# foobaz/pngloss

Measured on AMD Instinct MI355X. Metric: Mpixels/s (filter+quantise path), 4096x4096 RGBA8 s=19; bit-exact vs ref, higher is better.
Workload: dtype u8

## Files before the change

pngloss_amd/csrc/pl_seg_core.h:

```cpp
#ifndef PL_SEG_CORE_H
#define PL_SEG_CORE_H

#include <stdint.h>
#include <stddef.h>
#include <string.h>

#include "pl_result.h"

#if defined(__HIPCC__)
#define PLS_HD __host__ __device__ __forceinline__
#else
#define PLS_HD inline
#endif

#if defined(__HIP_DEVICE_COMPILE__)
#define PLS_THREADS(tid, nt) for (int tid = (int)threadIdx.x, pls_once_ = 1; pls_once_ && tid < (int)(nt); pls_once_ = 0)
#define PLS_SYNC() __syncthreads()
#define PLS_ATOMIC_ADD(p, v) atomicAdd((p), (v))
#define PLS_ATOMIC_MIN(p, v) atomicMin((p), (v))
#define PLS_ATOMIC_OR(p, v) atomicOr((p), (v))
#define PLS_ATOMIC_CAS(p, cmp, v) atomicCAS((p), (cmp), (v))
#define PLS_ATOMIC_ADD_RET(p, v) atomicAdd((p), (v))
#define PLS_ATOMIC_EXCH(p, v) atomicExch((p), (v))
#define PLS_ATOMIC_ADD64(p, v) atomicAdd((unsigned long long *)(p), (unsigned long long)(v))
#define PLS_CLOCK() wall_clock64()
#define PLS_ATOMIC_MAX(p, v) atomicMax((p), (v))
#define PLS_WAVE_LEADER(tid) (((tid) & 63) == 0)
__device__ __forceinline__ uint32_t pls_wave_sum_u32(uint32_t v) { for (int o = 32; o > 0; o >>= 1) v += __shfl_xor(v, o, 64); return v; }
__device__ __forceinline__ uint64_t pls_wave_sum_u64(uint64_t v) { for (int o = 32; o > 0; o >>= 1) v += __shfl_xor(v, o, 64); return v; }
__device__ __forceinline__ int pls_wave_max_i(int v) { for (int o = 32; o > 0; o >>= 1) { const int t = __shfl_xor(v, o, 64); v = t > v ? t : v; } return v; }
__device__ __forceinline__ int pls_wave_min_i(int v) { for (int o = 32; o > 0; o >>= 1) { const int t = __shfl_xor(v, o, 64); v = t < v ? t : v; } return v; }
#define PLS_ATOMIC_MAX_I(p, v) atomicMax((p), (v))
#define PLS_ATOMIC_MAX_U(p, v) atomicMax((p), (v))
#define PLS_ATOMIC_MIN_I(p, v) atomicMin((p), (v))
#define PLS_HOST_VISIBLE_ADD(p, v) __hip_atomic_fetch_add((p), (v), __ATOMIC_RELAXED, __HIP_MEMORY_SCOPE_SYSTEM)
#define PLS_HOST_VISIBLE_STORE(p, v) __hip_atomic_store((p), (v), __ATOMIC_RELAXED, __HIP_MEMORY_SCOPE_SYSTEM)
#else
#define PLS_THREADS(tid, nt) for (int tid = 0; tid < (int)(nt); ++tid)
#define PLS_SYNC() ((void)0)
#define PLS_ATOMIC_ADD(p, v) (*(p) += (v))
#define PLS_ATOMIC_MIN(p, v) (*(p) = *(p) < (v) ? *(p) : (v))
#define PLS_ATOMIC_OR(p, v) (*(p) |= (v))
inline uint32_t pls_host_cas(uint32_t *p, uint32_t cmp, uint32_t v) { const uint32_t old = *p; if (old == cmp) *p = v; return old; }
inline uint32_t pls_host_add_ret(uint32_t *p, uint32_t v) { const uint32_t old = *p; *p += v; return old; }
#define PLS_ATOMIC_CAS(p, cmp, v) pls_host_cas((p), (cmp), (v))
#define PLS_ATOMIC_ADD_RET(p, v) pls_host_add_ret((p), (v))
#define PLS_ATOMIC_EXCH(p, v) (*(p) = (v))
#define PLS_ATOMIC_ADD64(p, v) (*(p) += (v))
#define PLS_CLOCK() 0ull
#define PLS_ATOMIC_MAX(p, v) (*(p) = *(p) > (v) ? *(p) : (v))
#define PLS_WAVE_LEADER(tid) (true)
inline uint32_t pls_wave_sum_u32(uint32_t v) { return v; }
inline uint64_t pls_wave_sum_u64(uint64_t v) { return v; }
inline int pls_wave_max_i(int v) { return v; }
inline int pls_wave_min_i(int v) { return v; }
#define PLS_ATOMIC_MAX_I(p, v) (*(p) = *(p) > (v) ? *(p) : (v))
#define PLS_ATOMIC_MAX_U(p, v) (*(p) = *(p) > (v) ? *(p) : (v))
#define PLS_ATOMIC_MIN_I(p, v) (*(p) = *(p) < (v) ? *(p) : (v))
#define PLS_HOST_VISIBLE_ADD(p, v) (*(p) += (v))
#define PLS_HOST_VISIBLE_STORE(p, v) (*(p) = (v))
#endif

#if defined(__HIP_DEVICE_COMPILE__) && !defined(SEG_PLAIN_POINTERS)
#define SEG_AS_LDS __attribute__((address_space(3)))
#define SEG_AS_GLB __attribute__((address_space(1)))
#else
#define SEG_AS_LDS
#define SEG_AS_GLB
#endif
typedef SEG_AS_LDS uint32_t *seg_lds_u32;
typedef SEG_AS_LDS uint8_t *seg_lds_u8;
typedef SEG_AS_LDS uint16_t *seg_lds_u16;

#if defined(__HIPCC__)
#define PLS_UNROLL _Pragma("unroll")
#else
#define PLS_UNROLL
#endif
#define SEG_NFILT 5
#ifndef SEG_DEBUG_ROW
#define SEG_DEBUG_ROW(kind, failed, winner, start_none)
#endif
#ifndef SEG_DEBUG_REPAIR
#define SEG_DEBUG_REPAIR(f, c, sg, est, sid)
#endif
#ifndef SEG_DEBUG_BREAK
#define SEG_DEBUG_BREAK(f, c, sg, est, y)
#endif
#ifndef SEG_DEBUG_STATE
#define SEG_DEBUG_STATE(f, k, sl, i, ps)
// ... 609 lines not shown
    return true;
}
inline bool seg_build_params(SegParams &P, int strength, int bleed, bool force_seeded = false)
{
    memset(&P, 0, sizeof P);
    if (strength < 0 || strength > 255 || bleed < 1 || bleed > 32767) return false;
    P.strength = strength; P.bleed = bleed; P.unit = 1; P.tparts = SEG_TPARTS;
    for (int d = -256; d <= 255; d++) {
        const SegSplit s = seg_split_slow(d, bleed);
        P.lut_a[d + 256] = ((uint32_t)s.rem & 0xffffu) | ((uint32_t)s.h << 16);
        P.lut_b[d + 256] = ((uint32_t)s.t & 255u) | (((uint32_t)s.f & 255u) << 8) | (((uint32_t)s.v & 255u) << 16) | ((uint32_t)s.h << 24);
    }
    {
        int rm_ = 0, tm_ = 0;
        for (int D = 0; D < 256; D++) {
            const SegSplit a = seg_split_slow(D, bleed), b = seg_split_slow(-D, bleed);
            rm_ = seg_max(rm_, seg_max(seg_abs(a.rem), seg_abs(b.rem))); tm_ = seg_max(tm_, seg_max(seg_abs(a.h), seg_abs(b.h)));
            P.rt_max[D] = (uint8_t)seg_min(255, rm_ + tm_);
        }
    }
    int rmax = 0, tmax = 0;
    for (int d = -strength; d <= strength; d++) { const SegSplit s = seg_split_slow(d, bleed); if (seg_abs(s.rem) > rmax) rmax = seg_abs(s.rem); if (seg_abs(s.h) > tmax) tmax = seg_abs(s.h); }
    P.cmax = rmax + tmax; P.tmax = tmax; P.dmax = strength + P.cmax;
    if (!force_seeded && seg_build_exhaustive(P, strength, bleed)) return true;
    P.seeded = 1; P.kin = P.cmax <= 12 ? (bleed == 1 ? 20 : 16) : (P.cmax <= 24 ? 24 : SEG_KIN);
    P.ns = 0; P.nsp = 64; P.keyn = 0; P.ns_small = 0; P.small_ok = 0; P.idx0_big = P.idx0_small = (uint32_t)SEG_INVALID;
    if (P.cmax > 127 || tmax > 127 || 2 * P.cmax + 1 > SEG_NSP) return false;
    int tstep = 1;
    while ((2 * P.cmax + 1) * (2 * (tmax / tstep) + 1) > SEG_NSP) tstep++;
    int n = 0;
    for (int cn = -P.cmax; cn <= P.cmax; cn++)
        for (int th = -(tmax / tstep) * tstep; th <= tmax; th += tstep) P.seed_small[n++] = (uint32_t)(cn + 128) | ((uint32_t)(th + 128) << 8);
    P.nseed_small = n;
    return true;
}


#define SEG_SM_ENUM (SEG_TBL_WORDS * 4 + 2048 + SEG_SMALL_SEGS * SEG_L * 4 * 8 + 64 + 4 * 512 * 4 + 4 * 512 * 2 + 4 * SEG_NSP * 4 + 4 * SEG_NSP * 2 + SEG_THREADS * 2 + SEG_THREADS * 4 + 64)
#define SEG_SM_ENUM_NT(nt) (SEG_TBL_WORDS * 4 + (SEG_L + 1) * 4 * 8 + 2048 + 32 + 4 * SEG_HT * 4 + 4 * SEG_HT * 2 + 4 * SEG_NSP * 4 + 4 * SEG_NSP * 2 + (nt) * 2 + (nt) * 4 + 128)
#define SEG_SM_REPLAY (4096 + SEG_TBL_WORDS * 4 + SEG_GRP * SEG_L * 4 * 8 + SEG_GRP * 256 + SEG_GRP * SEG_PARTS * 4 * 8 + SEG_GRP * SEG_L * 16 + (SEG_GRP * SEG_L + 3) * 4 + 64)
#ifndef SEG_WATCH_OF
#define SEG_WATCH_OF(V) ((V) > 8 ? 2 : 8)
#endif
#define SEG_SM_POST_V(V) ((768 + ((V) + 1) * 256 + ((V) * SEG_L + 2) * 4 + 64 + 512 + 2 * ((V) * SEG_L + 2) + 2 * (V) * SEG_L + 32 + 64 + (V) * SEG_L + (V) * (SEG_L + 1) + SEG_WATCH_OF(V) * ((V) * (SEG_L + 1) + 8) + 2 * 20 * 4 + 512 + 64) * 4)
#define SEG_SM_POST SEG_SM_POST_V(SEG_VGRP)
#define SEG_SM_CTLVAL_V(V) (SEG_SM_CTL > SEG_SM_POST_V(V) ? SEG_SM_CTL : SEG_SM_POST_V(V))
#define SEG_SM_CTLVAL SEG_SM_CTLVAL_V(SEG_VGRP)
#define SEG_SM_CTL ((8 + 512 + (sizeof(SegCtl) + 7) / 8 * 2 + (sizeof(SegAcc) + 7) / 8 * 2 + 56 + SEG_NFILT * (SEG_COMMIT_W + 4) * 4 + SEG_COMMIT_W * 4 + (SEG_NFILT + 1) * 256 + 16) * 4)
static_assert((1024 + SEG_TBL_WORDS) * 4 <= SEG_SM_CTL, "a candidate workgroup of the control kernel (histograms + table staging) fits the commit workgroups' request");

PLS_HD void seg_cnt_add(uint32_t *cnt, int bin, uint32_t v) { PLS_ATOMIC_ADD(&cnt[bin >> 2], v << (8 * (bin & 3))); }
PLS_HD uint32_t seg_cnt_get(const uint32_t *cnt, int bin) { return (cnt[bin >> 2] >> (8 * (bin & 3))) & 255u; }
static_assert(SEG_L * 4 <= 255, "a segment's bump count of a bin fits a byte");
template <int F, bool TRX, int N = 0>
PLS_HD int seg_steps(const SegPix *px, int pstride, int n, SegState &st, const SegStepMem &M, const SegGeo &g, uint32_t *out, uint32_t *cnt)
{
    const int nn = N > 0 ? N : n;
    int bad = 0;
    if (nn <= 0) return 0;
    SegPix p = px[0];
    for (int k = 0; k < nn; k++) {
        const SegPix pn = px[(size_t)(k + 1 < nn ? k + 1 : k) * pstride];
        const uint32_t w = seg_step_fast<F, TRX>(p, st, bad, M, g);
        if (out) out[(size_t)k * 4] = w;
        if (cnt) seg_cnt_add(cnt, seg_cand_bin(w), 1u);
        p = pn;
    }
    return bad;
}
template <int F, bool TRX, int N = 0>
PLS_HD int seg_run_fast(const SegPix *px, int pstride, int n, SegState &st, seg_lds_cu32 tw, const SegGeo &g, seg_lds_cu32 lut)
{
    return seg_bad(seg_steps<F, TRX, N>(px, pstride, n, st, seg_step_mem(tw, lut), g, nullptr, nullptr)) ? 1 : 0;
}
template <bool TRX, int N = 0>
PLS_HD int seg_run_fast_t(int f, const SegPix *px, int pstride, int n, SegState &st, seg_lds_cu32 tw, const SegGeo &g, seg_lds_cu32 lut)
{
    switch (f) {
    case 1: return seg_run_fast<1, TRX, N>(px, pstride, n, st, tw, g, lut);
    case 2: return seg_run_fast<2, TRX, N>(px, pstride, n, st, tw, g, lut);
    case 3: return seg_run_fast<3, TRX, N>(px, pstride, n, st, tw, g, lut);
    case 4: return seg_run_fast<4, TRX, N>(px, pstride, n, st, tw, g, lut);
    default: return seg_run_fast<0, TRX, N>(px, pstride, n, st, tw, g, lut);
    }
}
PLS_HD int seg_run_fast_f(int f, bool trx, const SegPix *px, int pstride, int n, SegState &st, seg_lds_cu32 tw, const SegGeo &g, seg_lds_cu32 lut)
{
    return trx ? seg_run_fast_t<true>(f, px, pstride, n, st, tw, g, lut) : seg_run_fast_t<false>(f, px, pstride, n, st, tw, g, lut);
}
template <int N>
PLS_HD int seg_run_fast_f(int f, bool trx, const SegPix *px, int pstride, SegState &st, seg_lds_cu32 tw, const SegGeo &g, seg_lds_cu32 lut)
{
    static_assert(N > 0, "a compile-time count of steps");
    return trx ? seg_run_fast_t<true, N>(f, px, pstride, N, st, tw, g, lut) : seg_run_fast_t<false, N>(f, px, pstride, N, st, tw, g, lut);
}

#define SEG_K1 4
#ifndef SEG_K1_ONE_CHUNK
#define SEG_K1_ONE_CHUNK 4
#endif
PLS_HD int seg_k1(int ns) { return ns <= SEG_NSP ? SEG_K1_ONE_CHUNK : SEG_K1; }
#define SEG_HT 512
template <int NT, int K1>
PLS_HD void seg_enum_body_k(const SegJob &j, const SegParams &P, const SegCtlView &cv, int par, int f, int seg, int chalf, unsigned char *smem)
{
    static_assert(K1 > 0 && K1 < SEG_PL, "the dedupe lies inside the first part");
    if (cv.finished || cv.active != 1) return;
    const uint32_t W = j.W, bpp = j.bpp;
    constexpr int NCH = NT / SEG_NSP;
    const int c0 = chalf * NCH;
    if ((uint32_t)c0 >= bpp) return;
    const uint32_t x0 = (uint32_t)seg * SEG_L;
    if (x0 >= W) return;
    if (cv.start_x && x0 <= cv.start_x) return;
    uint32_t *tw = (uint32_t *)smem;
    SegPix *px = (SegPix *)(smem + SEG_TBL_WORDS * 4);
    uint32_t *lut = (uint32_t *)(px + (SEG_L + 1) * 4);
    uint32_t *trflag = lut + 512;
// ... 709 lines not shown
        }
        PLS_SYNC();
        PLS_THREADS(tid, NT) {
            const uint32_t total2 = misc[64 + NC];
            if ((uint32_t)tid < total2) {
                int k = 0;
                PLS_UNROLL
                for (int q = 1; q < NC; q++) k += (uint32_t)tid >= misc[64 + q] ? 1 : 0;
                const uint32_t i = (uint32_t)tid - misc[64 + k], cq = q0 + (uint32_t)k, u = cq / bpp, c = cq % bpp;
                SegState st = seg_state_unpack(pool2[misc[32 + k] + i]);
                const SegPix *pk = px + (size_t)k * NPX;
                const uint32_t sg0 = u * E, nsg = seg_umin(E, nseg - sg0);
                int bad = 0;
                for (uint32_t sl = 1; sl < nsg; sl++) {
                    const size_t slot = (((size_t)f * nseg + sg0 + sl) * 4 + c) * SEG_NSP + i;
                    for (int part = 0; part < SEG_PARTS; part++) {
                        if (part) j.rck[slot * (SEG_PARTS - 1) + (part - 1)] = bad ? 0xFFFFFFFFu : seg_state_pack(st);
                        bad |= seg_run_fast_f(f, trx, pk + 1 + sl * SEG_L + part * SEG_PL, 1, SEG_PL, st, SEG_LDS_CU32(tw), G, SEG_LDS_CU32(lut));
                    }
                    j.rst[slot] = bad ? 0xFFFFFFFFu : seg_state_pack(st);
                    SEG_DEBUG_STATE(f, (long)cv.y * 100000 + (long)cq, sl, i, bad ? 0xFFFFFFFFu : seg_state_pack(st));
                    if (sl + 1 == nsg) j.rout[slot] = (uint16_t)(bad ? (uint32_t)SEG_INVALID : seg_any_encode(P, f, pk[(sl + 1) * SEG_L], st));
                }
            }
        }
    }
    if (prof) {
        PLS_SYNC();
        PLS_THREADS(tid, NT) {
            if (tid == 0) {
                te[4] = PLS_CLOCK();
                for (int q = 0; q < PLR_SEG_ENUM_PHASES; q++) { PLS_ATOMIC_MAX(&j.result[PLR_SEG_ENUM_MAX + q], (int32_t)(te[q + 1] - te[q])); PLS_ATOMIC_ADD((uint32_t *)&j.result[PLR_SEG_ENUM_SUM + q], (uint32_t)(te[q + 1] - te[q])); }
                PLS_ATOMIC_ADD((uint32_t *)&j.result[PLR_SEG_ENUM_RUNS], 1u);
                PLS_ATOMIC_ADD((uint32_t *)&j.result[PLR_SEG_ENUM_STATES], 4u * misc[32 + NC] / (uint32_t)NC);
            }
        }
    }
}

PLS_HD bool seg_unit_from_seeds(const SegJob &j, const SegParams &P, const SegCtlView &cv, int f, int seeds)
{
    return seeds != 0 && P.seed_n > 0 && !seg_is_small(P, f) && cv.start_x == 0u && j.nbreak * 16u <= cv.y + 128u;
}

PLS_HD void seg_load_frozen(const SegJob &j, int par, int f, uint32_t *Hf, uint32_t *rank, int tid, int nt)
{
    for (int b = tid; b < 256; b += nt) {
        Hf[b] = j.H0[par * 256 + b] + j.base[((size_t)par * SEG_NFILT + f) * 256 + b];
        rank[b] = j.orig_rank[f * 256 + b];
    }
}

PLS_HD void seg_walk(int f, const SegPix *px, int pstride, uint32_t xa, uint32_t xe, SegState &st, seg_lds_cu32 tw, seg_lds_cu32 lut, const uint32_t *Hf,
                     const uint32_t *rank, const SegGeo &G, const uint32_t *lut_g, int bleed, uint32_t *out, uint32_t *cnt)
{
    const SegState st0 = st;
    int bad = 0;
    const SegStepMem M = seg_step_mem(tw, lut);
    const int n = xa < xe ? (int)(xe - xa) : 0;
    switch (f) {
    case 1: bad = seg_steps<1, true>(px, pstride, n, st, M, G, out, cnt); break;
    case 2: bad = seg_steps<2, true>(px, pstride, n, st, M, G, out, cnt); break;
    case 3: bad = seg_steps<3, true>(px, pstride, n, st, M, G, out, cnt); break;
    case 4: bad = seg_steps<4, true>(px, pstride, n, st, M, G, out, cnt); break;
    default: bad = seg_steps<0, true>(px, pstride, n, st, M, G, out, cnt); break;
    }
    if (seg_bad(bad)) {
        if (cnt && out) for (uint32_t x = xa; x < xe; x++) seg_cnt_add(cnt, seg_cand_bin(out[(size_t)(x - xa) * 4]), 0u - 1u);
        st = st0;
        for (uint32_t x = xa; x < xe; x++) {
            const uint32_t w = seg_step_scan(f, px[(size_t)(x - xa) * pstride], st, Hf, nullptr, rank, G, lut_g, bleed);
            if (out) out[(size_t)(x - xa) * 4] = w;
            if (cnt) seg_cnt_add(cnt, seg_cand_bin(w), 1u);
        }
    }
}

template <int NT, bool UNITS>
PLS_HD void seg_first_body(const SegJob &j, const SegParams &P, const SegCtlView &cv, int par, int f, unsigned char *smem)
{
    const SegCtl &ctl = j.ctl[par];
    if (cv.finished || cv.active != 1) return;
    const uint32_t W = j.W, bpp = j.bpp, nseg = j.nseg;
    const uint32_t sx = cv.start_x;
    if (sx >= W || sx == 0) return;
    const uint32_t first = sx / SEG_L;
    if (first + 1 >= nseg) return;
    const uint32_t E = UNITS ? seg_unit_of(P, f) : 1u, ulast = seg_umin((first / E) * E + E - 1u, nseg - 1u);
    const uint32_t wend = seg_umin(ulast, nseg - 2u);
    const uint32_t npix = (wend - first + 1u) * SEG_L;
    uint32_t *tw = (uint32_t *)smem;
    uint32_t *lut = tw + SEG_TBL_WORDS;
    uint32_t *Hf = lut + 512, *rank = Hf + 256;
    SegPix *px = (SegPix *)(rank + 256);
    const unsigned long long tf0 = (P.engine_flags & 1) ? PLS_CLOCK() : 0ull;
    const uint32_t y = cv.y;
    const uint32_t *row = seg_row_orig(j, y), *nab = y ? j.img + (size_t)(y - 1u) * W : nullptr, *e0g = seg_e0(j, y);
    const SegGeo G = seg_geo((int)cv.s);
    PLS_THREADS(tid, NT) {
        constexpr int NTW = (SEG_TBL_WORDS + NT - 1) / NT;
        uint32_t vt[NTW], vl = 0, vh = 0, vb = 0, vr = 0;
        SegPixRaw vp = seg_pix_raw_zero();
        PLS_UNROLL
        for (int q = 0; q < NTW; q++) { const int i = tid + q * NT; vt[q] = i < SEG_TBL_WORDS ? j.tables[(size_t)f * SEG_TBL_WORDS + i] : 0u; }
        if (tid < 512) vl = P.lut_a[tid];
        if (tid < 256) { const int b = tid; vh = j.H0[par * 256 + b]; vb = j.base[((size_t)par * SEG_NFILT + f) * 256 + b]; vr = j.orig_rank[f * 256 + b]; }
        static_assert(256 + SEG_UNIT * SEG_L <= NT, "a unit's pixels are staged by the threads behind the first 256");
        if (tid >= 256 && (uint32_t)(tid - 256) < npix) vp = seg_pix_fetch(row, nab, e0g, first * SEG_L + (uint32_t)(tid - 256), W);
        PLS_UNROLL
        for (int q = 0; q < NTW; q++) { const int i = tid + q * NT; if (i < SEG_TBL_WORDS) tw[i] = vt[q]; }
        if (tid < 512) lut[tid] = vl;
        if (tid < 256) { Hf[tid] = vh + vb; rank[tid] = vr; }
        if (tid >= 256 && (uint32_t)(tid - 256) < npix) seg_pix_split4(px + (tid - 256) * 4, vp, bpp, first * SEG_L + (uint32_t)(tid - 256), W);
    }
    PLS_SYNC();
    PLS_THREADS(tid, NT) {
        if (tid < 4 && (uint32_t)tid < bpp) {
            const int c = tid;
            SegState st = seg_state_unpack(ctl.state[f][c]);
            for (uint32_t sg = first; sg <= wend; sg++) {
                const uint32_t xa = sg == first ? sx : sg * SEG_L, xe = (sg + 1u) * SEG_L;
                seg_walk(f, px + (xa - first * SEG_L) * 4 + c, 4, xa, xe, st, SEG_LDS_CU32(tw), SEG_LDS_CU32(lut), Hf, rank, G, lut, P.bleed, nullptr, nullptr);
                if (sg + 1u <= ulast) {
                    j.entry[((size_t)f * nseg + sg + 1u) * 4 + c] = seg_state_pack(st);
                    j.dnout[((size_t)f * nseg + sg + 1u) * 4 + c] = (uint16_t)SEG_INVALID;
                }
// ... 440 lines not shown
PLS_HD int seg_none_reach(const SegJob &j, const SegParams &P, int s, int M, int m);

template <int CT>
PLS_HD void seg_extremes_body(const SegJob &j, const SegParams &P, const SegCtlView &cv, int par, unsigned char *smem)
{
    if (cv.finished || !j.rowmm) return;
    const uint32_t W = j.W, bpp = j.bpp, y = cv.y;
    const uint32_t *row = seg_row_orig(j, y), *e0g = seg_e0(j, y);
    uint32_t *mm = (uint32_t *)smem;
    PLS_THREADS(tid, CT) { if (tid == 0) { mm[0] = 0x80000000u ^ (uint32_t)(-(1 << 30)); mm[1] = 0x80000000u ^ (uint32_t)(1 << 30); } }
    PLS_SYNC();
    PLS_THREADS(tid, CT) {
        int vmax = -(1 << 30), vmin = 1 << 30;
        for (uint32_t x0 = (uint32_t)tid; x0 < W; x0 += 4u * CT) {
            uint32_t o[4], ea[4], eb[4];
            PLS_UNROLL
            for (int q = 0; q < 4; q++) { const uint32_t x = seg_umin(x0 + (uint32_t)q * CT, W - 1u); o[q] = row[x]; ea[q] = e0g[2 * (size_t)x]; eb[q] = e0g[2 * (size_t)x + 1]; }
            PLS_UNROLL
            for (int q = 0; q < 4; q++) {
                const uint32_t e[2] = { ea[q], eb[q] };
                const bool alpha0 = (bpp & 1u) == 0u && ((o[q] >> (8u * (bpp - 1u))) & 255u) == 0u;
                for (uint32_t c = 0; c < bpp; c++) {
                    if (alpha0 && c == bpp - 1u) continue;
                    const int v = (int)((o[q] >> (8 * c)) & 255u) + seg_err_plane(e, seg_plane_of_channel(bpp, (int)c));
                    vmax = seg_max(vmax, v); vmin = seg_min(vmin, v);
                }
            }
        }
        vmax = pls_wave_max_i(vmax); vmin = pls_wave_min_i(vmin);
        if (PLS_WAVE_LEADER(tid)) { PLS_ATOMIC_MAX_U(&mm[0], 0x80000000u ^ (uint32_t)vmax); PLS_ATOMIC_MIN(&mm[1], 0x80000000u ^ (uint32_t)vmin); }
    }
    PLS_SYNC();
    PLS_THREADS(tid, CT) { if (tid == 0) { SEG_AS_GLB int32_t *rmm = seg_rowmm(j, y); rmm[0] = (int)(mm[0] ^ 0x80000000u); rmm[1] = (int)(mm[1] ^ 0x80000000u); } }
}

template <int RNT>
PLS_HD void seg_replay_body(const SegJob &j, const SegParams &P, const SegCtlView &cv, int par, int f, int grp, unsigned char *smem)
{
    const SegCtl &ctl = j.ctl[par];
    if (cv.finished) return;
    const bool lazy = f == 0 && cv.active == 2;
    if (!lazy && cv.active != 1) return;
    const uint32_t W = j.W, bpp = j.bpp, nseg = j.nseg;
    const uint32_t sx = cv.start_x;
    const uint32_t first = sx / SEG_L;
    const uint32_t seg0 = (uint32_t)grp * SEG_GRP, x0g = seg0 * SEG_L;
    const bool walk = !lazy && sx < W && seg0 + SEG_GRP > first;
    uint32_t *Hf = (uint32_t *)smem, *rank = Hf + 256, *lut = Hf + 512, *tw = Hf + 1024;
    SegPix *px = (SegPix *)(tw + SEG_TBL_WORDS);
    uint32_t *cnt = (uint32_t *)(px + SEG_GRP * SEG_L * 4);
    uint32_t *lane = cnt + SEG_GRP * 64;
    uint32_t *cwl = lane + SEG_GRP * SEG_PARTS * 4 * 2;
    uint32_t *oaL = cwl + SEG_REPLAY_THREADS * 4;
    uint32_t *rm = tw;
    uint32_t *red = rm + 768;
    uint32_t *h0s = red + 16;
    const uint32_t y = cv.y;
    const uint32_t *row = seg_row_orig(j, y), *nab = y ? j.img + (size_t)(y - 1u) * W : nullptr, *e0g = seg_e0(j, y);
    const uint32_t *oab = y ? seg_row_orig(j, y - 1u) : nullptr;
    const SegGeo G = seg_geo((int)cv.s);
    const bool adaptive = !j.row_filters || y == 0;
    PLS_THREADS(tid, RNT) {
        const bool walker = walk && tid < SEG_GRP * SEG_PARTS * 4;
        const int sl = tid / (SEG_PARTS * 4), part = (tid >> 2) % SEG_PARTS, c = tid & 3;
        const uint32_t sg = seg0 + (uint32_t)sl;
        const bool live = walker && sg < nseg && sg >= first && (uint32_t)c < bpp;
        const size_t sc = ((size_t)f * nseg + (live ? sg : 0u)) * 4 + c;
        const uint32_t d = live ? (uint32_t)j.dnout[sc] : SEG_INVALID;
        constexpr int NTW = (SEG_TBL_WORDS + RNT - 1) / RNT;
        uint32_t vt[NTW], vl = 0, vh = 0, vb = 0, vr = 0;
        PLS_UNROLL
        for (int q = 0; q < NTW; q++) { const int i = tid + q * RNT; vt[q] = (walk && i < SEG_TBL_WORDS) ? j.tables[(size_t)f * SEG_TBL_WORDS + i] : 0u; }
        if (walk && tid < 512) vl = P.lut_a[tid];
        if (walk && tid < 256) { vh = j.H0[par * 256 + tid]; vb = j.base[((size_t)par * SEG_NFILT + f) * 256 + tid]; vr = j.orig_rank[f * 256 + tid]; }
        const bool pixlane = tid < SEG_REPLAY_THREADS;
        const uint32_t x = pixlane ? x0g + (uint32_t)tid : W;
        const SegPixRaw vp = seg_pix_fetch(row, nab, e0g, x, W);
        const uint32_t voa = (!lazy && oab && x < W) ? oab[x] : 0u;
        uint32_t voa0 = 0, vol0 = 0;
        SegVec16 vw, vw0; vw.a = vw.b = vw.c = vw.d = 0u; vw0 = vw;
        if (!lazy && tid == 0 && x0g) { voa0 = oab ? oab[x0g - 1] : 0u; vol0 = row[x0g - 1]; if (x0g <= sx) vw0 = *(const SEG_AS_GLB SegVec16 *)(j.cand + ((size_t)f * W + x0g - 1) * 4); }
        if (!lazy && x < W && (x < sx || !walk)) vw = *(const SEG_AS_GLB SegVec16 *)(j.cand + ((size_t)f * W + x) * 4);
        uint32_t ck[SEG_PARTS - 1], ent = 0;
        PLS_UNROLL
        for (int q = 0; q < SEG_PARTS - 1; q++) ck[q] = 0xFFFFFFFFu;
        if (live) {
            if (d != SEG_INVALID && d < SEG_NSP) {
                PLS_UNROLL
                for (int q = 0; q < SEG_PARTS - 1; q++) ck[q] = j.rck[(sc * SEG_NSP + d) * (SEG_PARTS - 1) + q];
            }
            if (part == 0) ent = sg == first ? ctl.state[f][c] : j.entry[sc];
        }
        uint32_t st0 = 0, range = 0xFFFFFFFFu;
        if (live) {
            const uint32_t x0 = sg * SEG_L, xend = (uint32_t)seg_min((int)(x0 + SEG_L), (int)W);
            bool mine = part == 0;
            uint32_t xa = sg == first ? sx : x0;
            if (part == 0) st0 = ent;
            else {
                uint32_t ckp = 0xFFFFFFFFu;
                PLS_UNROLL
                for (int q = 0; q < SEG_PARTS - 1; q++) if (q == part - 1) ckp = ck[q];
                if (ckp != 0xFFFFFFFFu && x0 + (uint32_t)part * SEG_PL < xend && x0 + (uint32_t)part * SEG_PL > xa) { mine = true; st0 = ckp; xa = x0 + (uint32_t)part * SEG_PL; }
            }
            if (mine) {
                uint32_t xe = xend;
                PLS_UNROLL
                for (int q = SEG_PARTS - 1; q >= 1; q--)
                    if (q > part && ck[q - 1] != 0xFFFFFFFFu && x0 + (uint32_t)q * SEG_PL < xend && x0 + (uint32_t)q * SEG_PL > xa) xe = x0 + (uint32_t)q * SEG_PL;
                range = (xa - x0g) | ((xe - x0g) << 16);
                SEG_DEBUG_COUNT(part ? 1 : 0, xe - xa);
            }
        }
        if (tid < SEG_GRP * SEG_PARTS * 4) { lane[2 * tid] = st0; lane[2 * tid + 1] = range; }
        if (walk) {
            PLS_UNROLL
            for (int q = 0; q < NTW; q++) { const int i = tid + q * RNT; if (i < SEG_TBL_WORDS) tw[i] = vt[q]; }
            if (tid < 512) lut[tid] = vl;
            if (tid < 256) { Hf[tid] = vh + vb; rank[tid] = vr; }
            for (int i = tid; i < SEG_GRP * 64; i += RNT) cnt[i] = 0u;
        }
        if (pixlane) {
            seg_pix_split4(px + tid * 4, vp, bpp, x, W);
            oaL[tid + 1] = voa;
            cwl[tid * 4 + 0] = vw.a; cwl[tid * 4 + 1] = vw.b; cwl[tid * 4 + 2] = vw.c; cwl[tid * 4 + 3] = vw.d;
        }
        if (tid == 0) {
            oaL[0] = voa0; oaL[SEG_REPLAY_THREADS + 1] = vol0;
            oaL[SEG_REPLAY_THREADS + 2] = (vw0.a & 255u) | ((vw0.b & 255u) << 8) | ((vw0.c & 255u) << 16) | ((vw0.d & 255u) << 24);
        }
    }
    PLS_SYNC();
    if (walk) {
        PLS_THREADS(tid, RNT) {
            if (tid < SEG_GRP * SEG_PARTS * 4 && lane[2 * tid + 1] != 0xFFFFFFFFu) {
                const int sl = tid / (SEG_PARTS * 4), c = tid & 3;
                SegState st = seg_state_unpack(lane[2 * tid]);
                const uint32_t ra = lane[2 * tid + 1] & 0xffffu, re = lane[2 * tid + 1] >> 16;
                seg_walk(f, px + ra * 4 + c, 4, x0g + ra, x0g + re, st, SEG_LDS_CU32(tw), SEG_LDS_CU32(lut), Hf, rank, G, lut, P.bleed, cwl + ra * 4 + c, cnt + sl * 64);
            }
        }
        PLS_SYNC();
    }
    SegAcc &A = j.acc[par];
    PLS_THREADS(tid, RNT) { if (tid < 16) red[tid] = tid == 14 ? (0x80000000u ^ (uint32_t)(-(1 << 30))) : (tid == 15 ? (0x80000000u ^ (uint32_t)(1 << 30)) : 0u); }
    PLS_SYNC();
    {
        PLS_THREADS(tid, RNT) {
            if (walk && tid >= RNT - SEG_REPLAY_THREADS && tid < RNT - SEG_REPLAY_THREADS + 256) {
                const int b = tid - (RNT - SEG_REPLAY_THREADS);
                uint32_t tot = 0, cvs[SEG_GRP];
                PLS_UNROLL
                for (int sl = 0; sl < SEG_GRP; sl++) cvs[sl] = seg_cnt_get(cnt + sl * 64, b);
                PLS_UNROLL
                for (int sl = 0; sl < SEG_GRP; sl++) {
                    const uint32_t sg = seg0 + (uint32_t)sl;
                    if (sg < nseg && sg >= first) { j.segcnt[((size_t)f * nseg + sg) * 256 + b] = (uint16_t)cvs[sl]; tot += cvs[sl]; }
                }
                j.grpcnt[((size_t)f * j.ngrp + grp) * 256 + b] = tot;
            }
            const uint32_t x = (!lazy && tid < SEG_REPLAY_THREADS) ? x0g + (uint32_t)tid : W;
            uint64_t derr = 0; uint32_t hs[SEG_NFILT] = { 0, 0, 0, 0, 0 };
            if (x < W) {
                SegVec16 w; w.a = cwl[tid * 4 + 0]; w.b = cwl[tid * 4 + 1]; w.c = cwl[tid * 4 + 2]; w.d = cwl[tid * 4 + 3];
                if (walk && x >= sx) *(SEG_AS_GLB SegVec16 *)(j.cand + ((size_t)f * W + x) * 4) = w;
                uint32_t lw[4];
                if (tid) { PLS_UNROLL for (int c = 0; c < 4; c++) lw[c] = cwl[(tid - 1) * 4 + c] & 255u; }
                else {
                    uint32_t l0 = 0;
                    if (x0g && x0g <= sx) l0 = oaL[SEG_REPLAY_THREADS + 2];
                    else if (x0g) {
                        for (uint32_t c = 0; c < bpp; c++) l0 |= (walk ? (lane[2 * c] & 255u) : 0u) << (8 * c);
                        j.grpleft[(size_t)f * j.ngrp + grp] = l0;
                    }
                    PLS_UNROLL for (int c = 0; c < 4; c++) lw[c] = (l0 >> (8 * c)) & 255u;
                }
                const uint32_t wv[4] = { w.a, w.b, w.c, w.d };
                const uint32_t oav4 = oaL[tid + 1], odv4 = oaL[tid];
                for (uint32_t c = 0; c < bpp; c++) {
                    const int sh = 8 * (int)c;
                    const SegPix pc = px[tid * 4 + c];
                    const int back = (int)(wv[c] & 255u), nl = x ? (int)lw[c] : 0;
                    const int ov = (int)(pc.w & 255u), nav = (int)((pc.w >> 8) & 255u), ndv = (int)((pc.w >> 16) & 255u);
                    const int olv = tid ? (int)(px[(tid - 1) * 4 + c].w & 255u) : (int)((oaL[SEG_REPLAY_THREADS + 1] >> sh) & 255u);
                    const int oav = (int)((oav4 >> sh) & 255u), odv = (int)((odv4 >> sh) & 255u);
                    const int da = (oav - ov) - (nav - back), dd = (odv - ov) - (ndv - back), dl = (olv - ov) - (nl - back);
                    const uint32_t wgt = (bpp <= 2 && c == 0) ? 3u : 1u;
                    derr += (uint64_t)(wgt * (uint32_t)(da * da + dd * dd + dl * dl));
                    if (adaptive) {
                        const int preds[SEG_NFILT] = { 0, nl, nav, (nav + nl) >> 1, seg_paeth(nav, ndv, nl) };
                        for (int g = 0; g < SEG_NFILT; g++) { const int bb = (back - preds[g]) & 255; hs[g] += (uint32_t)(bb < 128 ? bb : 256 - bb); }
                    }
                }
            }
            derr = (uint64_t)pls_wave_sum_u32((uint32_t)derr);
            if (adaptive) for (int g = 0; g < SEG_NFILT; g++) hs[g] = pls_wave_sum_u32(hs[g]);
            if (PLS_WAVE_LEADER(tid)) {
                PLS_ATOMIC_ADD64((uint64_t *)&red[0], derr);
                if (adaptive) for (int g = 0; g < SEG_NFILT; g++) PLS_ATOMIC_ADD(&red[2 + g], hs[g]);
            }
        }
    }
    int R = -1;
    if (f == 0 && j.rowmm) {
        const int32_t *rmm = seg_rowmm(j, y);
        PLS_THREADS(tid, RNT) {
            if (tid == 0) red[12] = (uint32_t)seg_none_reach(j, P, (int)cv.s, rmm[0], rmm[1]);
            if (tid >= 64 && tid < 64 + 256) h0s[tid - 64] = j.H0[par * 256 + (tid - 64)];
        }
        PLS_SYNC();
        R = (int)red[12];
        if (R >= 0) {
            PLS_THREADS(tid, RNT) {
                for (int i = tid; i < 768; i += RNT) {
                    const int centre = i - 256;
                    const int lo = seg_min(seg_max(centre - R, 0), 255), hi = seg_min(seg_max(centre + R, 0), 255);
                    uint32_t m = 0;
                    for (int b = lo; b <= hi; b += 8) {
                        uint32_t h[8];
                        PLS_UNROLL
                        for (int q = 0; q < 8; q++) h[q] = h0s[seg_min(b + q, hi)];
                        PLS_UNROLL
                        for (int q = 0; q < 8; q++) m = h[q] > m ? h[q] : m;
                    }
                    rm[i] = m;
                }
            }
            PLS_SYNC();
            PLS_THREADS(tid, RNT) {
                uint64_t lb = 0;
                const uint32_t rowbumps = W * bpp;
                const uint32_t x = tid < SEG_REPLAY_THREADS ? x0g + (uint32_t)tid : W;
                if (x < W) {
                    for (uint32_t c = 0; c < bpp; c++) {
                        const SegPix pc = px[tid * 4 + c];
                        uint32_t hmax;
                        if (pc.w >> 24) hmax = h0s[0];
                        else hmax = rm[seg_min(seg_max((int)(pc.w & 255u) + pc.e0, -256), 511) + 256];
                        const uint32_t fr = hmax + rowbumps;
                        lb += 33u + (uint32_t)__builtin_clz(fr ? fr : 1u);
                    }
                }
                lb = pls_wave_sum_u64(lb);
                if (PLS_WAVE_LEADER(tid) && lb) PLS_ATOMIC_ADD64((uint64_t *)&red[10], lb);
            }
        }
    }
    PLS_SYNC();
    PLS_THREADS(tid, RNT) {
        if (tid == 0) {
            if (!lazy) {
                PLS_ATOMIC_ADD64(&A.derr[f], *(uint64_t *)&red[0]);
                if (adaptive) for (int g = 0; g < SEG_NFILT; g++) PLS_ATOMIC_ADD(&A.hs[f][g], red[2 + g]);
            }
            if (f == 0 && R >= 0) { PLS_ATOMIC_ADD64(&A.none_lb, *(uint64_t *)&red[10]); PLS_ATOMIC_ADD(&A.lb_valid, 1u); }
        }
    }
}

struct SegVal {
    const uint32_t *cw, *ro, *na, *e0, *lut, *H0, *rank, *cum;
    uint32_t bpp, sx, xg0, W;
    int f, bleed;
    SegGeo G;
    uint32_t *wbits;
    const uint8_t *slot_of;
    const uint32_t *pcw;
    uint32_t pc_stride;
    uint8_t *binb;
    const uint32_t *btop;
    const uint32_t *hiG, *loG;
};
#define SEG_BINB_STRIDE (SEG_L * 4 + 4)
#define SEG_PC_SEG (SEG_L + 1)
#define SEG_PC_STRIDE_V(V) ((V) * SEG_PC_SEG + 8)
#define SEG_NBAND 20
PLS_HD uint32_t seg_pc_get(const uint32_t *pcw, uint32_t pc_stride, uint32_t slot, int d)
{
    const uint32_t w = pcw[(size_t)slot * pc_stride + (d / (SEG_L * 4)) * SEG_PC_SEG + ((d % (SEG_L * 4)) >> 2)];
    return (w >> (8 * (d & 3))) & 255u;
}
PLS_HD int seg_validate_one(const SegVal &V, int d, int mode)
{
    const int c = d & 3, k = d >> 2;
    const uint32_t x = V.xg0 + (uint32_t)k, bpp = V.bpp;
    const int sl = k / SEG_L;
    const uint32_t w0 = V.cw[(k + 2) * 4 + c], w1 = V.cw[(k + 1) * 4 + c], w2 = V.cw[k * 4 + c];
    if (mode == 0) V.binb[sl * SEG_BINB_STRIDE + (d - sl * SEG_L * 4)] = (uint8_t)seg_cand_bin(w0);
    if (x >= V.W || x < V.sx || (uint32_t)c >= bpp) return 1;
    const uint32_t o = V.ro[k + 1];
    const int pe0 = seg_err_plane(V.e0 + 2 * k, seg_plane_of_channel(bpp, c));
    const bool trp = (bpp & 1u) == 0u && (uint32_t)c == bpp - 1u && ((o >> (8u * (bpp - 1u))) & 255u) == 0u;
    int rem1, thr1, rem2, thr2;
    seg_rem_thr(V.lut, V.bleed, x >= 1 ? seg_cand_diff(w1) : 0, rem1, thr1);
    seg_rem_thr(V.lut, V.bleed, x >= 2 ? seg_cand_diff(w2) : 0, rem2, thr2);
    const int left = x >= 1 ? seg_cand_byte(w1) : 0, cn = rem1 + thr2;
    const int orig = (int)((o >> (8 * c)) & 255u), above = (int)((V.na[k + 1] >> (8 * c)) & 255u), diag = x ? (int)((V.na[k] >> (8 * c)) & 255u) : 0;
    const int pred = seg_predict(V.f, above, diag, left);
    const int back = seg_cand_byte(w0), diff = seg_cand_diff(w0), bin = seg_cand_bin(w0);
    if (trp) return (back == 0 && diff == 0 && bin == ((0 - pred) & 255)) ? 1 : 0;
    const int osym = seg_sext8(orig - pred), lo = osym - orig;
    const int filt = osym + seg_sext16(pe0 + cn);
    const SegBand bd = seg_band(filt, lo, V.G);
    const int v = back + lo;
    if (!(v >= bd.v0 && v <= bd.v1 && diff == seg_sext16(filt - v) && bin == (v & 255))) return 0;
    if (bd.v0 == bd.v1) return 1;
// ... 873 lines not shown
```

Before: 93.61.

## Fuse distortion-error accumulation and candidate stores into the segment walk

The walker threads now accumulate squared distortion error inline while stepping pixels, and write candidate words straight to global memory during the walk. The separate per-pixel replay pass is skipped for walked pixels when no adaptive histogram is needed. A boundary fixup adjusts for the left-neighbour value at segment starts. This removes a second pass over the row and a barrier, at the cost of more per-step work and scattered global stores from walkers, plus more complex correctness bookkeeping for bit-exactness.

```diff
diff --git a/pngloss_amd/csrc/pl_seg_core.h b/pngloss_amd/csrc/pl_seg_core.h
--- a/pngloss_amd/csrc/pl_seg_core.h
+++ b/pngloss_amd/csrc/pl_seg_core.h
@@ -14,6 +14,7 @@
 #endif
 
 #if defined(__HIP_DEVICE_COMPILE__)
+#define PLS_ASSUME(c) __builtin_assume(c)
 #define PLS_THREADS(tid, nt) for (int tid = (int)threadIdx.x, pls_once_ = 1; pls_once_ && tid < (int)(nt); pls_once_ = 0)
 #define PLS_SYNC() __syncthreads()
 #define PLS_ATOMIC_ADD(p, v) atomicAdd((p), (v))
@@ -36,6 +37,7 @@
 #define PLS_HOST_VISIBLE_ADD(p, v) __hip_atomic_fetch_add((p), (v), __ATOMIC_RELAXED, __HIP_MEMORY_SCOPE_SYSTEM)
 #define PLS_HOST_VISIBLE_STORE(p, v) __hip_atomic_store((p), (v), __ATOMIC_RELAXED, __HIP_MEMORY_SCOPE_SYSTEM)
 #else
+#define PLS_ASSUME(c) ((void)0)
 #define PLS_THREADS(tid, nt) for (int tid = 0; tid < (int)(nt); ++tid)
 #define PLS_SYNC() ((void)0)
 #define PLS_ATOMIC_ADD(p, v) (*(p) += (v))
@@ -751,8 +753,19 @@
 PLS_HD void seg_cnt_add(uint32_t *cnt, int bin, uint32_t v) { PLS_ATOMIC_ADD(&cnt[bin >> 2], v << (8 * (bin & 3))); }
 PLS_HD uint32_t seg_cnt_get(const uint32_t *cnt, int bin) { return (cnt[bin >> 2] >> (8 * (bin & 3))) & 255u; }
 static_assert(SEG_L * 4 <= 255, "a segment's bump count of a bin fits a byte");
+struct SegErrSink { seg_lds_cu32 oa; int sh, odv, olv, nl; uint32_t sum; };
+PLS_HD uint32_t seg_err_weight(uint32_t bpp, int c) { return (bpp <= 2 && c == 0) ? 3u : 1u; }
+PLS_HD void seg_err_add(SegErrSink &e, uint32_t pw, uint32_t w, uint32_t oaw)
+{
+    const int ov = (int)(pw & 255u), nav = (int)((pw >> 8) & 255u), ndv = (int)((pw >> 16) & 255u), back = (int)(w & 255u);
+    const int oav = (int)((oaw >> e.sh) & 255u);
+    const int da = (oav - ov) - (nav - back), dd = (e.odv - ov) - (ndv - back), dl = (e.olv - ov) - (e.nl - back);
+    e.sum += (uint32_t)(seg_mul24(da, da) + seg_mul24(dd, dd) + seg_mul24(dl, dl));
+    e.odv = oav; e.olv = ov; e.nl = back;
+}
 template <int F, bool TRX, int N = 0>
-PLS_HD int seg_steps(const SegPix *px, int pstride, int n, SegState &st, const SegStepMem &M, const SegGeo &g, uint32_t *out, uint32_t *cnt)
+PLS_HD int seg_steps(const SegPix *px, int pstride, int n, SegState &st, const SegStepMem &M, const SegGeo &g, uint32_t *out, uint32_t *cnt, SegErrSink *err = nullptr,
+                     SEG_AS_GLB uint32_t *gout = nullptr)
 {
     const int nn = N > 0 ? N : n;
     int bad = 0;
@@ -760,9 +773,12 @@
     SegPix p = px[0];
     for (int k = 0; k < nn; k++) {
         const SegPix pn = px[(size_t)(k + 1 < nn ? k + 1 : k) * pstride];
+        const uint32_t oaw = err ? err->oa[k] : 0u;
         const uint32_t w = seg_step_fast<F, TRX>(p, st, bad, M, g);
         if (out) out[(size_t)k * 4] = w;
+        if (gout) gout[(size_t)k * 4] = w;
         if (cnt) seg_cnt_add(cnt, seg_cand_bin(w), 1u);
+        if (err) seg_err_add(*err, p.w, w, oaw);
         p = pn;
     }
     return bad;
@@ -1578,26 +1594,32 @@
 }
 
 PLS_HD void seg_walk(int f, const SegPix *px, int pstride, uint32_t xa, uint32_t xe, SegState &st, seg_lds_cu32 tw, seg_lds_cu32 lut, const uint32_t *Hf,
-                     const uint32_t *rank, const SegGeo &G, const uint32_t *lut_g, int bleed, uint32_t *out, uint32_t *cnt)
+                     const uint32_t *rank, const SegGeo &G, const uint32_t *lut_g, int bleed, uint32_t *out, uint32_t *cnt, SegErrSink *err = nullptr,
+                     SEG_AS_GLB uint32_t *gout = nullptr)
 {
     const SegState st0 = st;
+    const SegErrSink err0 = err ? *err : SegErrSink();
     int bad = 0;
     const SegStepMem M = seg_step_mem(tw, lut);
     const int n = xa < xe ? (int)(xe - xa) : 0;
     switch (f) {
-    case 1: bad = seg_steps<1, true>(px, pstride, n, st, M, G, out, cnt); break;
-    case 2: bad = seg_steps<2, true>(px, pstride, n, st, M, G, out, cnt); break;
-    case 3: bad = seg_steps<3, true>(px, pstride, n, st, M, G, out, cnt); break;
-    case 4: bad = seg_steps<4, true>(px, pstride, n, st, M, G, out, cnt); break;
-    default: bad = seg_steps<0, true>(px, pstride, n, st, M, G, out, cnt); break;
+    case 1: bad = seg_steps<1, true>(px, pstride, n, st, M, G, out, cnt, err, gout); break;
+    case 2: bad = seg_steps<2, true>(px, pstride, n, st, M, G, out, cnt, err, gout); break;
+    case 3: bad = seg_steps<3, true>(px, pstride, n, st, M, G, out, cnt, err, gout); break;
+    case 4: bad = seg_steps<4, true>(px, pstride, n, st, M, G, out, cnt, err, gout); break;
+    default: bad = seg_steps<0, true>(px, pstride, n, st, M, G, out, cnt, err, gout); break;
     }
     if (seg_bad(bad)) {
         if (cnt && out) for (uint32_t x = xa; x < xe; x++) seg_cnt_add(cnt, seg_cand_bin(out[(size_t)(x - xa) * 4]), 0u - 1u);
         st = st0;
+        if (err) *err = err0;
         for (uint32_t x = xa; x < xe; x++) {
-            const uint32_t w = seg_step_scan(f, px[(size_t)(x - xa) * pstride], st, Hf, nullptr, rank, G, lut_g, bleed);
+            const SegPix p = px[(size_t)(x - xa) * pstride];
+            const uint32_t w = seg_step_scan(f, p, st, Hf, nullptr, rank, G, lut_g, bleed);
             if (out) out[(size_t)(x - xa) * 4] = w;
+            if (gout) gout[(size_t)(x - xa) * 4] = w;
             if (cnt) seg_cnt_add(cnt, seg_cand_bin(w), 1u);
+            if (err) seg_err_add(*err, p.w, w, err->oa[x - xa]);
         }
     }
 }
@@ -2144,6 +2166,7 @@
     uint32_t *lane = cnt + SEG_GRP * 64;
     uint32_t *cwl = lane + SEG_GRP * SEG_PARTS * 4 * 2;
     uint32_t *oaL = cwl + SEG_REPLAY_THREADS * 4;
+    uint32_t *sums = oaL + SEG_REPLAY_THREADS + 4;
     uint32_t *rm = tw;
     uint32_t *red = rm + 768;
     uint32_t *h0s = red + 16;
@@ -2152,6 +2175,9 @@
     const uint32_t *oab = y ? seg_row_orig(j, y - 1u) : nullptr;
     const SegGeo G = seg_geo((int)cv.s);
     const bool adaptive = !j.row_filters || y == 0;
+    const bool pixpass = !lazy && (adaptive || !walk || sx > x0g);
+    const bool direct = walk && !pixpass && !(f == 0 && j.rowmm);
+    static_assert((SEG_SM_REPLAY - 64) % 8 == 4 && SEG_SM_REPLAY - 64 + 4 + 8 * 4 <= SEG_SM_REPLAY, "the row sums lie on an even word inside the request's last 64 bytes");
     PLS_THREADS(tid, RNT) {
         const bool walker = walk && tid < SEG_GRP * SEG_PARTS * 4;
         const int sl = tid / (SEG_PARTS * 4), part = (tid >> 2) % SEG_PARTS, c = tid & 3;
@@ -2221,22 +2247,37 @@
             oaL[0] = voa0; oaL[SEG_REPLAY_THREADS + 1] = vol0;
             oaL[SEG_REPLAY_THREADS + 2] = (vw0.a & 255u) | ((vw0.b & 255u) << 8) | ((vw0.c & 255u) << 16) | ((vw0.d & 255u) << 24);
         }
+        if (tid < 8) sums[tid] = 0u;
     }
     PLS_SYNC();
     if (walk) {
         PLS_THREADS(tid, RNT) {
+            uint32_t es = 0;
             if (tid < SEG_GRP * SEG_PARTS * 4 && lane[2 * tid + 1] != 0xFFFFFFFFu) {
                 const int sl = tid / (SEG_PARTS * 4), c = tid & 3;
                 SegState st = seg_state_unpack(lane[2 * tid]);
                 const uint32_t ra = lane[2 * tid + 1] & 0xffffu, re = lane[2 * tid + 1] >> 16;
-                seg_walk(f, px + ra * 4 + c, 4, x0g + ra, x0g + re, st, SEG_LDS_CU32(tw), SEG_LDS_CU32(lut), Hf, rank, G, lut, P.bleed, cwl + ra * 4 + c, cnt + sl * 64);
+                SegErrSink E;
+                E.oa = SEG_LDS_CU32(oaL + ra + 1); E.sh = 8 * c; E.sum = 0u;
+                E.odv = (int)((oaL[ra] >> E.sh) & 255u);
+                E.olv = ra ? (int)(px[(ra - 1) * 4 + c].w & 255u) : (int)((oaL[SEG_REPLAY_THREADS + 1] >> E.sh) & 255u);
+                E.nl = (x0g + ra) ? st.left : 0;
+                SEG_AS_GLB uint32_t *gw = j.cand + ((size_t)f * W + x0g + ra) * 4 + c;
+                PLS_ASSUME(gw != nullptr);
+                seg_walk(f, px + ra * 4 + c, 4, x0g + ra, x0g + re, st, SEG_LDS_CU32(tw), SEG_LDS_CU32(lut), Hf, rank, G, lut, P.bleed, cwl + ra * 4 + c, cnt + sl * 64, &E, gw);
+                es = seg_err_weight(bpp, c) * E.sum;
+            }
+            if (tid < SEG_GRP * SEG_PARTS * 4) {
+                es = pls_wave_sum_u32(es);
+                if (PLS_WAVE_LEADER(tid) && es) {
+                    if (direct) PLS_ATOMIC_ADD64(&j.acc[par].derr[f], (uint64_t)es);
+                    else PLS_ATOMIC_ADD64((uint64_t *)&sums[0], (uint64_t)es);
+                }
             }
         }
         PLS_SYNC();
     }
     SegAcc &A = j.acc[par];
-    PLS_THREADS(tid, RNT) { if (tid < 16) red[tid] = tid == 14 ? (0x80000000u ^ (uint32_t)(-(1 << 30))) : (tid == 15 ? (0x80000000u ^ (uint32_t)(1 << 30)) : 0u); }
-    PLS_SYNC();
     {
         PLS_THREADS(tid, RNT) {
             if (walk && tid >= RNT - SEG_REPLAY_THREADS && tid < RNT - SEG_REPLAY_THREADS + 256) {
@@ -2251,20 +2292,32 @@
                 }
                 j.grpcnt[((size_t)f * j.ngrp + grp) * 256 + b] = tot;
             }
-            const uint32_t x = (!lazy && tid < SEG_REPLAY_THREADS) ? x0g + (uint32_t)tid : W;
+            if (walk && tid == 0 && x0g > sx && x0g < W) {
+                uint32_t l0 = 0;
+                for (uint32_t c = 0; c < bpp; c++) l0 |= (lane[2 * c] & 255u) << (8 * c);
+                j.grpleft[(size_t)f * j.ngrp + grp] = l0;
+            }
+            if (walk && tid < SEG_GRP * SEG_PARTS * 4) {
+                const uint32_t rg = lane[2 * tid + 1], ra = (rg != 0xFFFFFFFFu && (rg & 0xffffu)) ? (rg & 0xffffu) : 1u;
+                const int c = tid & 3;
+                const int nls = (int)(lane[2 * tid] & 255u), nlw = (int)(cwl[(ra - 1) * 4 + c] & 255u);
+                const int back = (int)(cwl[ra * 4 + c] & 255u), dlo = (int)(px[(ra - 1) * 4 + c].w & 255u) - (int)(px[ra * 4 + c].w & 255u) + back;
+                int64_t fix = (int64_t)((dlo - nlw) * (dlo - nlw) - (dlo - nls) * (dlo - nls)) * (int64_t)seg_err_weight(bpp, c);
+                if (rg == 0xFFFFFFFFu || !(rg & 0xffffu)) fix = 0;
+                if (fix) PLS_ATOMIC_ADD64(&A.derr[f], (uint64_t)fix);
+            }
+            if (!pixpass) continue;
+            const uint32_t x = tid < SEG_REPLAY_THREADS ? x0g + (uint32_t)tid : W;
             uint64_t derr = 0; uint32_t hs[SEG_NFILT] = { 0, 0, 0, 0, 0 };
-            if (x < W) {
+            const bool unwalked = !walk || x < sx;
+            if (x < W && (adaptive || unwalked)) {
                 SegVec16 w; w.a = cwl[tid * 4 + 0]; w.b = cwl[tid * 4 + 1]; w.c = cwl[tid * 4 + 2]; w.d = cwl[tid * 4 + 3];
-                if (walk && x >= sx) *(SEG_AS_GLB SegVec16 *)(j.cand + ((size_t)f * W + x) * 4) = w;
                 uint32_t lw[4];
                 if (tid) { PLS_UNROLL for (int c = 0; c < 4; c++) lw[c] = cwl[(tid - 1) * 4 + c] & 255u; }
                 else {
                     uint32_t l0 = 0;
                     if (x0g && x0g <= sx) l0 = oaL[SEG_REPLAY_THREADS + 2];
-                    else if (x0g) {
-                        for (uint32_t c = 0; c < bpp; c++) l0 |= (walk ? (lane[2 * c] & 255u) : 0u) << (8 * c);
-                        j.grpleft[(size_t)f * j.ngrp + grp] = l0;
-                    }
+                    else if (x0g) { for (uint32_t c = 0; c < bpp; c++) l0 |= (walk ? (lane[2 * c] & 255u) : 0u) << (8 * c); }
                     PLS_UNROLL for (int c = 0; c < 4; c++) lw[c] = (l0 >> (8 * c)) & 255u;
                 }
                 const uint32_t wv[4] = { w.a, w.b, w.c, w.d };
@@ -2277,8 +2330,8 @@
                     const int olv = tid ? (int)(px[(tid - 1) * 4 + c].w & 255u) : (int)((oaL[SEG_REPLAY_THREADS + 1] >> sh) & 255u);
                     const int oav = (int)((oav4 >> sh) & 255u), odv = (int)((odv4 >> sh) & 255u);
                     const int da = (oav - ov) - (nav - back), dd = (odv - ov) - (ndv - back), dl = (olv - ov) - (nl - back);
-                    const uint32_t wgt = (bpp <= 2 && c == 0) ? 3u : 1u;
-                    derr += (uint64_t)(wgt * (uint32_t)(da * da + dd * dd + dl * dl));
+                    const uint32_t wgt = seg_err_weight(bpp, (int)c);
+                    if (unwalked) derr += (uint64_t)(wgt * (uint32_t)(da * da + dd * dd + dl * dl));
                     if (adaptive) {
                         const int preds[SEG_NFILT] = { 0, nl, nav, (nav + nl) >> 1, seg_paeth(nav, ndv, nl) };
                         for (int g = 0; g < SEG_NFILT; g++) { const int bb = (back - preds[g]) & 255; hs[g] += (uint32_t)(bb < 128 ? bb : 256 - bb); }
@@ -2288,16 +2341,17 @@
             derr = (uint64_t)pls_wave_sum_u32((uint32_t)derr);
             if (adaptive) for (int g = 0; g < SEG_NFILT; g++) hs[g] = pls_wave_sum_u32(hs[g]);
             if (PLS_WAVE_LEADER(tid)) {
-                PLS_ATOMIC_ADD64((uint64_t *)&red[0], derr);
-                if (adaptive) for (int g = 0; g < SEG_NFILT; g++) PLS_ATOMIC_ADD(&red[2 + g], hs[g]);
-            }
-        }
-    }
+                if (derr) PLS_ATOMIC_ADD64((uint64_t *)&sums[0], derr);
+                if (adaptive) for (int g = 0; g < SEG_NFILT; g++) PLS_ATOMIC_ADD(&sums[2 + g], hs[g]);
+            }
+        }
+    }
+    if (direct) return;
     int R = -1;
     if (f == 0 && j.rowmm) {
         const int32_t *rmm = seg_rowmm(j, y);
         PLS_THREADS(tid, RNT) {
-            if (tid == 0) red[12] = (uint32_t)seg_none_reach(j, P, (int)cv.s, rmm[0], rmm[1]);
+            if (tid == 0) { red[10] = red[11] = 0u; red[12] = (uint32_t)seg_none_reach(j, P, (int)cv.s, rmm[0], rmm[1]); }
             if (tid >= 64 && tid < 64 + 256) h0s[tid - 64] = j.H0[par * 256 + (tid - 64)];
         }
         PLS_SYNC();
@@ -2342,8 +2396,8 @@
     PLS_THREADS(tid, RNT) {
         if (tid == 0) {
             if (!lazy) {
-                PLS_ATOMIC_ADD64(&A.derr[f], *(uint64_t *)&red[0]);
-                if (adaptive) for (int g = 0; g < SEG_NFILT; g++) PLS_ATOMIC_ADD(&A.hs[f][g], red[2 + g]);
+                PLS_ATOMIC_ADD64(&A.derr[f], *(uint64_t *)&sums[0]);
+                if (adaptive) for (int g = 0; g < SEG_NFILT; g++) PLS_ATOMIC_ADD(&A.hs[f][g], sums[2 + g]);
             }
             if (f == 0 && R >= 0) { PLS_ATOMIC_ADD64(&A.none_lb, *(uint64_t *)&red[10]); PLS_ATOMIC_ADD(&A.lb_valid, 1u); }
         }
```

Result: slower. 89.93 (-3.9%).
